# dingodb/dingo-store

Hardware: AMD Instinct MI355X
Metric: QPS @ recall@10, IVF-Flat 10Mx768 nprobe=32 (higher is better)
Workload: dtype f32; 1 GPU; IVF-Flat 10M x 768 fp32 nlist=4096 nprobe=32 batch=1024 k=10; n=10000000, d=768, nlist=4096, nprobe=32, batch=1024, k=10, parallelism=single GPU

## Files before the change

### dingo-store_amd/csrc/dg_abi.cpp

```cpp
#include <cmath>
#include <cstdarg>
#include <cstdio>
#include <cstring>
#include <algorithm>
#include <functional>
#include <atomic>
#include <vector>

#include "dg_internal.h"
#include "dg_sq8_core.h"

static thread_local char g_err[1024] = "";

void dg_set_error(const char* fmt, ...) {
  va_list ap;
  va_start(ap, fmt);
  vsnprintf(g_err, sizeof(g_err), fmt, ap);
  va_end(ap);
}

extern "C" void dg_last_error(char* buf, int64_t len) {
  if (buf && len > 0) {
    strncpy(buf, g_err, len - 1);
    buf[len - 1] = 0;
// ... 20 lines not shown
  }
  g_alloc_gen.fetch_add(1, std::memory_order_relaxed);
  size_t newcap = std::max(bytes, b.cap + b.cap / 2);
  void* np = nullptr;
  if (hipMalloc(&np, newcap) != hipSuccess) {
    dg_set_error("hipMalloc(%zu) failed", newcap);
    return DG_ENOMEM;
  }
  if (keep && b.p && b.bytes) {
    if (hipMemcpyAsync(np, b.p, b.bytes, hipMemcpyDeviceToDevice, s) !=
        hipSuccess) {
      (void)hipFree(np);
      dg_set_error("grow copy failed");
      return DG_EINTERNAL;
    }
  }
  if (b.p) {
    (void)hipStreamSynchronize(s);
    (void)hipFree(b.p);
  }
  b.p = np;
  b.cap = newcap;
  b.bytes = bytes;
  return DG_OK;
}

static bool scan_fused_enabled() {
  const char* e = getenv("DG_SCAN_FUSED");
  return !(e && e[0] == '0' && e[1] == '\0');
}

static bool scan_mfma_enabled() {
  const char* e = getenv("DG_SCAN_MFMA");
  return !(e && e[0] == '0' && e[1] == '\0');
}

static int32_t scan_pair_py() {
  const char* e = getenv("DG_SCAN_PAIR");
  if (e && e[0] && e[1] == '\0') {
    if (e[0] == '0') return 0;
    if (e[0] == '1' || e[0] == '2' || e[0] == '4') return e[0] - '0';
  }
  return dg_index::kScanPairPY;
}

static int32_t scan_f16_py(int32_t mean_probes) {
  const char* e = getenv("DG_SCAN_F16_PY");
  if (e && e[0] && e[1] == '\0' &&
      (e[0] == '1' || e[0] == '2' || e[0] == '4'))
    return e[0] - '0';
  return std::min(4, std::max(1, (mean_probes + 7) / 8));
}

static int64_t range_span_blocks() {
  const char* e = getenv("DG_RANGE_SPAN_BLOCKS");
  const long long v = e ? atoll(e) : 0;
  return v > 0 ? std::min<long long>(v, 1ll << 30) : 1ll << 30;
}

static void dbuf_free(dg_dbuf& b) {
  if (b.p) (void)hipFree(b.p);
  b = {};
}

struct DbufGuard {
  dg_dbuf& b;
// ... 1994 lines not shown
    }
    if (!ix->capturing) (void)hipEventRecord(ix->ev[3], ix->stream);
    if (st == DG_OK) {
      uint64_t* result = slab;
      if (slab_k > k) {
        dgk::fill_base_total(ix->stream, nq, slab_k, bt, bt + nq);
        dgk::select_u64(ix->stream, slab, bt, bt + nq, nq, k, final_tk, k);
        result = final_tk;
      }
      dgk::emit_results(ix->stream, result, (const int64_t*)ix->d_csr_ids.p,
                        dqn, nq, k, emit_metric,
                        metric == DG_METRIC_L2 ? 1 : 0, d_out_dist,
                        d_out_ids);
    }
    if (!ix->capturing) (void)hipEventRecord(ix->ev[4], ix->stream);
    ix->times.last_scan_bytes_alg =
        is_bin ? (int64_t)ix->ntotal * (ix->d_user / 8)
               : (int64_t)ix->ntotal * (d * 4 + 4);
  } else {
    int32_t np = nprobe > 0 ? nprobe : 80;
    np = std::min(np, nlist);
    if ((st = dbuf_reserve(ix->ws_dots, (size_t)nq * nlist * 4, ix->stream,
                           false)) != DG_OK ||
        (st = dbuf_reserve(ix->ws_probes,
                           (size_t)nq * np * 12 + (size_t)nq * k * 8,
                           ix->stream, false)) != DG_OK) {
      return st;
    }
    uint64_t* coarse_tk = (uint64_t*)ix->ws_probes.p;
    int32_t* probes = (int32_t*)(coarse_tk + (size_t)nq * np);
    uint64_t* final_tk = (uint64_t*)(probes + (size_t)nq * np);
    const uint8_t* maskp =
        ix->has_mask ? (const uint8_t*)ix->d_list_mask.p : nullptr;
    if (is_pq && np == nlist) {
      st = sgemm_dots(ix, dq, nq, (const float*)ix->d_centroids.p, nlist, d,
                      (float*)ix->ws_dots.p);
      if (st != DG_OK) {
        return st;
      }
    }
    if (np == nlist) {
      dgk::probes_all(ix->stream, nq, np, maskp, probes);
    } else {
      if (np > 2048) {
        dg_set_error("nprobe %d > 2048 (and < nlist) unsupported", np);
        return DG_ENOT_SUPPORT;
      }
      st = dots(dq, nq, ix->d_centroids.p, nlist, (float*)ix->ws_dots.p);
      if (st != DG_OK) {
        return st;
      }
      const int cmode = is_bin ? 0 : metric == DG_METRIC_L2 ? 1 : 2;
      const int32_t nseg_c = (int32_t)std::min<int64_t>(
          16, std::max<int64_t>(1, nlist / 8192));
      if (nseg_c > 1) {
        dg_dbuf& seg = ix->ws_seg;
        if ((st = dbuf_reserve(seg,
                               (size_t)nq * nseg_c * np * 8 +
                                   (size_t)nq * 2 * 8,
                               ix->stream, false)) != DG_OK)
          return st;
        uint64_t* seg_slab = (uint64_t*)seg.p;
        int64_t* bt_c = (int64_t*)(seg_slab + (size_t)nq * nseg_c * np);
        dgk::select_dense(ix->stream, (const float*)ix->ws_dots.p,
                          (const float*)ix->d_cnorms.p, nq, nlist, nlist,
                          nseg_c, np, cmode, nullptr, 0, seg_slab,
                          (int64_t)nseg_c * np, 0);
        dgk::fill_base_total(ix->stream, nq, (int64_t)nseg_c * np, bt_c,
                             bt_c + nq);
        dgk::select_u64(ix->stream, seg_slab, bt_c, bt_c + nq, nq, np,
                        coarse_tk, np);
      } else {
        dgk::select_dense(ix->stream, (const float*)ix->ws_dots.p,
                          (const float*)ix->d_cnorms.p, nq, nlist, nlist, 1,
                          np, cmode, nullptr, 0, coarse_tk, np, 0);
      }
      dgk::probe_unpack(ix->stream, coarse_tk, nq, np, maskp, probes);
    }
    if (!ix->capturing) (void)hipEventRecord(ix->ev[1], ix->stream);

    size_t inv_bytes = (size_t)nlist * 4 * 3 + ((size_t)nlist + 1) * 12 +
                       (size_t)nq * np * 8 * 2 + ((size_t)nq + 1) * 8 * 2 +
                       (size_t)nq * np * 8 + 64;
    if ((st = dbuf_reserve(ix->ws_inv, inv_bytes, ix->stream, false)) !=
        DG_OK) {
      return st;
    }
    char* wp = (char*)ix->ws_inv.p;
    int32_t* inv_counts = (int32_t*)wp;            wp += (size_t)nlist * 4;
    int32_t* cursors = (int32_t*)wp;               wp += (size_t)nlist * 4;
    wp += (size_t)nlist * 4;
    int64_t* inv_offsets64 = (int64_t*)wp;         wp += ((size_t)nlist + 1) * 8;
    int32_t* inv_offsets32 = (int32_t*)wp;         wp += ((size_t)nlist + 1) * 4;
    int32_t* inv_q = (int32_t*)wp;                 wp += (size_t)nq * np * 4;
    int32_t* inv_rank = (int32_t*)wp;              wp += (size_t)nq * np * 4;
    int64_t* qp_off = (int64_t*)wp;                wp += (size_t)nq * np * 8;
    int64_t* q_total = (int64_t*)wp;               wp += (size_t)nq * 8;
    int64_t* q_cand_base = (int64_t*)wp;

    int64_t* sscr = scan_scratch(ix, &st);
    if (st != DG_OK) {
      return st;
    }
    (void)hipMemsetAsync(inv_counts, 0, (size_t)nlist * 4, ix->stream);
    dgk::hist_probes(ix->stream, probes, nq, np, nlist, inv_counts);
    dgk::excl_scan_i32_to_i64(ix->stream, inv_counts, nlist, inv_offsets64,
                              sscr);
    dgk::init_cursors(ix->stream, inv_offsets64, nlist + 1, inv_offsets32);
    dgk::init_cursors(ix->stream, inv_offsets64, nlist, cursors);
    dgk::scatter_probes(ix->stream, probes, nq, np, nullptr, cursors, inv_q,
                        inv_rank);
    const int32_t chunk_rows = dg_index::kChunkRows;
    const int64_t ub_cand =
        nq * ix->h_len_prefix_desc[std::min<int32_t>(np, nlist)];
    const int64_t partial_per_q =
        (int64_t)np * ix->cpl_max * (chunk_rows / 256) * k;
    const bool fused = !is_pq && !is_bin && !rr &&
                       k <= dg_index::kScanFuseMaxK &&
                       nq * partial_per_q <= ub_cand && scan_fused_enabled();
    ix->last_scan_fused = fused;
    const bool is_f16 = !is_pq && !is_bin && ix->storage == DG_STORAGE_F16;
    ix->last_scan_f16 = is_f16;
    const bool is_sq8 = !is_pq && !is_bin && ix->storage == DG_STORAGE_SQ8;
    ix->last_scan_sq8 = is_sq8;
    if (is_sq8 &&
        (st = dbuf_reserve(ix->ws_sq8q, (size_t)nq * d * 4 + (size_t)nq * 4,
                           ix->stream, false)) != DG_OK)
      return st;
    const bool mfma = fused && (is_f16 || is_sq8 || scan_mfma_enabled());
    ix->last_scan_mfma = mfma;
    const int32_t pair_py =
        mfma && !is_f16 && !is_sq8 && dg_scan_pair_applies((int32_t)d, nq)
            ? scan_pair_py()
            : 0;
    ix->last_scan_pair = pair_py > 0;
    if (pair_py > 0 &&
        (st = dbuf_reserve(ix->ws_qimage,
                           (size_t)dg_scan_qimage_bytes(nq, (int32_t)d),
                           ix->stream, false)) != DG_OK) {
      return st;
    }
    if (fused) {
// ... 130 lines not shown
                          inv_offsets32, inv_q, inv_rank, qp_off, q_cand_base,
                          np, metric, d_bitmap, chunk_rows,
                          (uint64_t*)ix->ws_cand.p, mean_probes);
    }
    if (!ix->capturing) (void)hipEventRecord(ix->ev[3], ix->stream);

    if (rr) {
      if ((st = build_thr(is_bin)) == DG_OK) {
        dgk::count_below(ix->stream, (const uint64_t*)ix->ws_cand.p,
                         q_cand_base, q_total, d_thr, emit_metric, dqn,
                         rr->radius, nq, d_rcounts);
        st = range_finish([&](const int64_t*, int64_t* d_cursors,
                              uint64_t* d_out) -> dg_status {
          dg_dbuf d_off2{};
          dg_status s3 = dbuf_reserve(d_off2, ((size_t)nq + 1) * 8,
                                      ix->stream, false);
          if (s3 != DG_OK) return s3;
          (void)hipMemcpyAsync(d_off2.p, rr->lims, ((size_t)nq + 1) * 8,
                               hipMemcpyHostToDevice, ix->stream);
          dgk::compact_below(ix->stream, (const uint64_t*)ix->ws_cand.p,
                             q_cand_base, q_total, d_thr, emit_metric, dqn,
                             rr->radius, (const int64_t*)d_off2.p, nq,
                             d_cursors, d_out);
          (void)hipStreamSynchronize(ix->stream);
          dbuf_free(d_off2);
          return DG_OK;
        });
      }
      (void)hipEventRecord(ix->ev[4], ix->stream);
      ix->times.last_nq = nq;
      return st;
    }
    if (fused) {
      dgk::fill_base_total(ix->stream, nq, partial_per_q, q_cand_base,
                           q_total);
      dgk::select_u64(ix->stream, (const uint64_t*)ix->ws_partial.p,
                      q_cand_base, q_total, nq, k, final_tk, k);
    } else {
      dgk::select_u64(ix->stream, (const uint64_t*)ix->ws_cand.p, q_cand_base,
                      q_total, nq, k, final_tk, k);
    }
    dgk::emit_results(ix->stream, final_tk, (const int64_t*)ix->d_csr_ids.p,
                      dqn, nq, k, emit_metric, metric == DG_METRIC_L2 ? 1 : 0,
                      d_out_dist, d_out_ids);
    if (!ix->capturing) (void)hipEventRecord(ix->ev[4], ix->stream);
  }
  ix->times.last_nq = nq;
  return st;
}


static dg_status search_device_impl(dg_index* ix, int64_t nq,
                                    const float* d_x, int32_t k,
                                    int32_t nprobe, const dg_filter* filter,
                                    float* d_out_dist, int64_t* d_out_ids,
                                    bool binary_entry, const char* fn,
                                    bool may_capture = true) {
  if (!ix || !d_x || !d_out_dist || !d_out_ids || nq <= 0) {
    dg_set_error("bad search args");
    return DG_EINVAL;
  }
  if (!entry_matches(ix, binary_entry, fn)) return DG_EINVAL;
  if (binary_entry && nq > kMaxScanLen) {
    dg_set_error("nq %lld > %d per call unsupported", (long long)nq,
                 kMaxScanLen);
    return DG_EINVAL;
  }
  if (k <= 0) return DG_OK;
  if (k > 2048) {
    dg_set_error("k > 2048 not supported");
// ... 3 lines not shown
  if (!ix->is_ready() || ix->ntotal == 0 ||
      (ix->desc.kind == DG_INDEX_IVF_PQ && !ix->pq_trained)) {
    std::shared_lock lk(ix->rw);
    (void)hipMemsetAsync(d_out_dist, 0, (size_t)nq * k * 4, ix->stream);
    (void)hipMemsetAsync(d_out_ids, 0xff, (size_t)nq * k * 8, ix->stream);
    return DG_OK;
  }
  {
    std::unique_lock lk(ix->rw, std::defer_lock);
    if (!ix->csr_valid) {
      lk.lock();
      if (!ix->csr_valid) {
        dg_status st = finalize_csr(ix);
        if (st != DG_OK) return st;
      }
    }
  }
  std::shared_lock lk(ix->rw);
  std::lock_guard sg(ix->search_mu);

  const bool graph_ok = nq <= 4 && k <= 128 &&
                        ix->desc.kind == DG_INDEX_IVF_FLAT &&
                        (!filter || filter->kind == DG_FILTER_NONE) &&
                        getenv("DG_NO_GRAPH") == nullptr;
  if (graph_ok) {
    const uint64_t gen =
        ix->index_gen + g_alloc_gen.load(std::memory_order_relaxed);
    const size_t q_bytes = (size_t)nq * ix->d_user * 4;
    const size_t dist_bytes = (size_t)nq * k * 4;
    const size_t ids_bytes = (size_t)nq * k * 8;
    const bool fused_now = scan_fused_enabled();
    const bool mfma_now = scan_mfma_enabled();
    const int32_t pair_now = scan_pair_py();
    if (ix->graph_exec && ix->graph_nq == (int32_t)nq &&
        ix->graph_k == k && ix->graph_np == nprobe &&
        ix->graph_fused == fused_now && ix->graph_mfma == mfma_now &&
        ix->graph_pair == pair_now &&
        ix->graph_gen == gen) {
      DG_HIP_CHECK(hipMemcpyAsync(ix->ws_gq.p, d_x, q_bytes,
                                  hipMemcpyDeviceToDevice, ix->stream));
      DG_HIP_CHECK(hipGraphLaunch(ix->graph_exec, ix->stream));
      DG_HIP_CHECK(hipMemcpyAsync(d_out_dist, ix->ws_gout.p, dist_bytes,
                                  hipMemcpyDeviceToDevice, ix->stream));
      DG_HIP_CHECK(hipMemcpyAsync(
          d_out_ids, (char*)ix->ws_gout.p + dist_bytes, ids_bytes,
          hipMemcpyDeviceToDevice, ix->stream));
      ix->times.last_nq = 0;
      return DG_OK;
    }
    if (!may_capture)
      return search_core(ix, nq, d_x, k, nprobe, filter, d_out_dist,
                         d_out_ids);
    dg_status st = search_core(ix, nq, d_x, k, nprobe, filter, d_out_dist,
                               d_out_ids);
    if (st != DG_OK) return st;
    if (dbuf_reserve(ix->ws_gq, q_bytes, ix->stream, false) != DG_OK ||
        dbuf_reserve(ix->ws_gout, dist_bytes + ids_bytes, ix->stream,
                     false) != DG_OK)
      return DG_OK;
    if (ix->graph_exec) {
      (void)hipGraphExecDestroy(ix->graph_exec);
      ix->graph_exec = nullptr;
    }
    std::unique_lock cl(ix->capture_mu);
    (void)hipStreamSynchronize(ix->stream);
    const uint64_t gen2 =
        ix->index_gen + g_alloc_gen.load(std::memory_order_relaxed);
    ix->capturing = true;
    hipGraph_t graph = nullptr;
    bool captured = false;
    if (hipStreamBeginCapture(ix->stream, hipStreamCaptureModeThreadLocal) ==
        hipSuccess) {
      dg_status cst = search_core(
          ix, nq, (const float*)ix->ws_gq.p, k, nprobe, nullptr,
          (float*)ix->ws_gout.p,
          (int64_t*)((char*)ix->ws_gout.p + dist_bytes));
      if (hipStreamEndCapture(ix->stream, &graph) == hipSuccess &&
          cst == DG_OK && graph) {
        hipGraphExec_t ge = nullptr;
        if (hipGraphInstantiate(&ge, graph, nullptr, nullptr, 0) ==
            hipSuccess) {
          ix->graph_exec = ge;
          ix->graph_nq = (int32_t)nq;
          ix->graph_k = k;
          ix->graph_np = nprobe;
          ix->graph_fused = fused_now;
          ix->graph_mfma = mfma_now;
          ix->graph_pair = pair_now;
          ix->graph_gen = gen2;
          captured = true;
        }
      }
      if (graph) (void)hipGraphDestroy(graph);
    }
    if (!captured) (void)hipGetLastError();
    ix->capturing = false;
    return DG_OK;
  }
  return search_core(ix, nq, d_x, k, nprobe, filter, d_out_dist, d_out_ids);
}

extern "C" dg_status dg_search_device(dg_index* ix, int64_t nq,
                                      const float* d_x, int32_t k,
                                      int32_t nprobe, const dg_filter* filter,
                                      float* d_out_dist, int64_t* d_out_ids) {
  return search_device_impl(ix, nq, d_x, k, nprobe, filter, d_out_dist,
                            d_out_ids, false, "dg_search_device");
}

extern "C" dg_status dg_search_binary_device(dg_index* ix, int64_t nq,
                                             const uint8_t* d_x, int32_t k,
                                             int32_t nprobe,
                                             const dg_filter* filter,
                                             float* d_out_dist,
                                             int64_t* d_out_ids) {
  return search_device_impl(ix, nq, (const float*)d_x, k, nprobe, filter,
                            d_out_dist, d_out_ids, true,
                            "dg_search_binary_device");
}

dg_status dg_search_device_flush(dg_index* ix, int64_t nq, const void* d_x,
// ... 449 lines not shown
        for (size_t i = 0; i < c && st == DG_OK; i++)
          if (ibuf[i] >= 0) ix->id_count.emplace(ibuf[i], 1);
      }
      ix->ntotal = ntotal;
      ix->n_deleted = ndel;
      ix->csr_valid = false;
  ix->index_gen++;
    }
  } while (0);
  fclose(f);
  if (st != DG_OK) {
    dg_index_destroy(ix);
    return st;
  }
  ix->trained = trained != 0;
  *out = ix;
  return DG_OK;
}

extern "C" void dg_lock_write(dg_index* ix) {
  if (ix) ix->rw.lock();
}

extern "C" void dg_unlock_write(dg_index* ix) {
  if (ix) ix->rw.unlock();
}

extern "C" int dg_last_scan_fused(dg_index* ix) {
  if (!ix) return 0;
  std::lock_guard sg(ix->search_mu);
  return ix->last_scan_fused ? 1 : 0;
}

extern "C" int dg_last_scan_pair(dg_index* ix) {
  if (!ix) return 0;
  std::lock_guard sg(ix->search_mu);
  return ix->last_scan_pair ? 1 : 0;
}

extern "C" int dg_last_scan_sq8(dg_index* ix) {
  if (!ix) return 0;
  std::lock_guard sg(ix->search_mu);
  return ix->last_scan_sq8 ? 1 : 0;
}

extern "C" int dg_last_scan_mfma(dg_index* ix) {
  if (!ix) return 0;
  std::lock_guard sg(ix->search_mu);
  return ix->last_scan_mfma ? 1 : 0;
}

extern "C" dg_status dg_stats(dg_index* ix, dg_stats_out* out) {
  if (!ix || !out) return DG_EINVAL;
  std::shared_lock lk(ix->rw);
  DeviceGuard g(ix->device);
  memset(out, 0, sizeof(*out));
  out->ntotal = ix->ntotal - ix->n_deleted;
  out->d = ix->d_user;
  out->metric = ix->desc.metric;
  out->kind = ix->desc.kind;
  out->nlist = ix->desc.nlist;
  out->is_trained = ix->is_ready() ? 1 : 0;
  size_t db = 0;
  for (auto b : {&ix->d_vectors, &ix->d_ids, &ix->d_assign, &ix->d_centroids,
                 &ix->d_cnorms, &ix->d_csr_offsets, &ix->d_csr_vectors,
                 &ix->d_csr_ids, &ix->d_csr_vnorms, &ix->d_csr_t,
// ... 35 lines not shown
```

### dingo-store_amd/csrc/dg_internal.h

```cpp
#pragma once

#include <hip/hip_fp16.h>
#include <hip/hip_runtime.h>
#include <rocblas/rocblas.h>

#include <atomic>
#include <cstdint>
#include <cstdio>
#include <mutex>
#include <shared_mutex>
#include <string>
#include <unordered_map>
#include <vector>

#include "../../include/dingo_gpu.h"
#include "dg_scan_split.h"

#define DG_HIP_CHECK(expr)                                              \
  do {                                                                  \
    hipError_t _e = (expr);                                             \
    if (_e != hipSuccess) {                                             \
      dg_set_error("HIP error %s at %s:%d: %s", hipGetErrorName(_e),    \
                   __FILE__, __LINE__, hipGetErrorString(_e));          \
      return DG_EINTERNAL;                                              \
    }                                                                   \
  } while (0)

#define DG_ROCBLAS_CHECK(expr)                                          \
  do {                                                                  \
    rocblas_status _s = (expr);                                         \
    if (_s != rocblas_status_success) {                                 \
      dg_set_error("rocBLAS error %d at %s:%d", (int)_s, __FILE__,      \
                   __LINE__);                                           \
      return DG_EINTERNAL;                                              \
    }                                                                   \
  } while (0)

void dg_set_error(const char* fmt, ...);

dg_status dg_ingest_rows(dg_index* ix, int64_t n, const int64_t* ids,
                         const float* x, const uint8_t* codes,
                         const int32_t* assign);

dg_status dg_ingest_bits(dg_index* ix, int64_t n, const int64_t* ids,
                         const uint8_t* bits, const int32_t* assign);

dg_status dg_search_device_flush(dg_index* ix, int64_t nq, const void* d_x,
                                 int32_t k, int32_t nprobe,
// ... 84 lines not shown
  dg_dbuf d_csr_t;
  dg_dbuf d_chunk_meta;
  int32_t total_chunks = 0;
  static constexpr int32_t kChunkRows = 1024;
  static constexpr int32_t kScanFuseMaxK = 64;
  static constexpr int32_t kScanPairPY = 2;
  int32_t cpl_max = 0;


  bool pq_trained = false;
  dg_dbuf d_codebooks;
  dg_dbuf d_codes;
  dg_dbuf d_csr_codes;
  dg_dbuf d_S;
  dg_dbuf d_cb_norms;
  dg_dbuf ws_T;
  dg_dbuf ws_Tf32;

  dg_dbuf d_list_mask;
  bool has_mask = false;

  std::unordered_map<int64_t, int32_t> id_count;

  dg_dbuf ws_queries, ws_qnorms, ws_dots, ws_probes, ws_inv, ws_cand,
      ws_units, ws_small, ws_topk;
  dg_dbuf ws_scan;
  dg_dbuf ws_seg;
  dg_dbuf ws_bm;
  dg_dbuf ws_partial;
  bool last_scan_fused = false;
  bool last_scan_mfma = false;
  bool last_scan_pair = false;
  dg_dbuf ws_qimage;

  hipEvent_t ev[12] = {};
  dg_stage_times times;
  bool events_ready = false;

  hipGraphExec_t graph_exec = nullptr;
  int32_t graph_nq = 0, graph_k = 0, graph_np = 0;
  bool graph_fused = false;
  bool graph_mfma = false;
  int32_t graph_pair = 0;
  uint64_t graph_gen = 0;
  uint64_t index_gen = 1;
  dg_dbuf ws_gq, ws_gout;
  bool capturing = false;

  std::atomic<dg_batcher*> batcher{nullptr};

  std::shared_mutex rw;
  std::mutex search_mu;
  std::shared_mutex capture_mu;
};

namespace dgk {
void probe_unpack(hipStream_t s, const uint64_t* topk, int64_t nq,
                  int32_t nprobe, const uint8_t* mask, int32_t* probes);
void probes_all(hipStream_t s, int64_t nq, int32_t nprobe,
                const uint8_t* mask, int32_t* probes);
void init_cursors(hipStream_t s, const int64_t* offsets, int32_t n,
                  int32_t* cursors);
void select_dense(hipStream_t s, const float* scores, const float* cnorms,
                  int64_t rows, int64_t cols, int64_t ld, int32_t nseg,
                  int32_t k, int mode, const uint32_t* bitmap,
                  int64_t col_base, uint64_t* out, int64_t out_stride,
                  int64_t out_offset);
int select_dense_threads(int32_t k);
void select_u64(hipStream_t s, const uint64_t* cand, const int64_t* base,
                const int64_t* total, int64_t nq, int32_t k, uint64_t* out,
                int64_t out_stride);
void gather_rows_by_index(hipStream_t s, const float* src, const int64_t* idx,
                          int64_t n, int32_t d, float* dst);
void fill_base_total(hipStream_t s, int64_t nq, int64_t len, int64_t* base,
                     int64_t* total);
void tombstone(hipStream_t s, const int64_t* pos, int64_t n, int64_t* ids);
void hamming_dists(hipStream_t s, const uint32_t* X, int64_t nq,
                   const uint32_t* Y, int64_t cols, int32_t wp, float* out,
                   int64_t ld);
void hamming_range(hipStream_t s, bool compact, const uint32_t* X, int64_t nq,
                   const uint32_t* Y, int64_t cols, int32_t wp,
                   const uint32_t* bitmap, int32_t radius, int64_t* counts,
                   const int64_t* lims, int64_t* cursors, uint64_t* out,
                   int64_t max_blocks );
void argmin_score(hipStream_t s, const float* scores, int64_t n, int32_t cols,
                  int32_t* out);
void transpose_chunks_u32(hipStream_t s, const uint32_t* units,
                          int32_t n_units, const int64_t* csr_offsets,
                          const int32_t* chunk_off, const int64_t* chunk_base,
                          const uint32_t* rowmajor, int32_t wp,
                          int32_t chunk_rows, uint32_t* twords);
void bivf_scan(hipStream_t s, const uint32_t* units, int32_t n_units,
               const int64_t* csr_offsets, const int32_t* chunk_off,
               const int64_t* chunk_base, const uint32_t* twords,
               const uint32_t* queries, int32_t wp,
               const int32_t* inv_offsets, const int32_t* inv_q,
               const int32_t* inv_rank, const int64_t* qp_off,
               const int64_t* q_cand_base, int32_t nprobe,
               const uint32_t* bitmap, int32_t chunk_rows, uint64_t* cand);
void bits_to_pm1(hipStream_t s, const uint32_t* x, int64_t n, int32_t d,
                 int32_t wp, float* out);
void binarise(hipStream_t s, const float* c, int64_t n, int32_t d, int32_t wp,
              uint32_t* out);
void row_norms(hipStream_t s, const float* x, int64_t n, int32_t d,
               float* out);
void normalize_rows(hipStream_t s, float* x, int64_t n, int32_t d);
void argmin_rows(hipStream_t s, const float* dots, const float* cnorms,
                 int64_t n, int32_t nlist, int metric, int32_t* out);
// ... 168 lines not shown
```

### dingo-store_amd/csrc/kernels.hip.cpp

```cpp
#include <hip/hip_fp16.h>
#include <hip/hip_runtime.h>

#include <cstdint>

#include "dg_internal.h"
#include "dg_shard_core.h"
#include "dg_sq8_core.h"

#define WAVE 64

__device__ __forceinline__ uint32_t enc_f32(float x) {
  uint32_t u = __float_as_uint(x);
  return (int32_t)u < 0 ? ~u : (u | 0x80000000u);
}
__device__ __forceinline__ float dec_f32(uint32_t e) {
  uint32_t u = (e & 0x80000000u) ? (e & 0x7fffffffu) : ~e;
  return __uint_as_float(u);
}
__device__ __forceinline__ uint64_t pack_cand(float key, uint32_t row) {
  return ((uint64_t)enc_f32(key) << 32) | row;
}
static constexpr uint64_t kCandEmpty = ~0ull;

__global__ void k_iota_i32(int32_t* p, int64_t n, int32_t v) {
// ... 115 lines not shown
__device__ void topk_merge_block(uint64_t* lds, int32_t k, int32_t cnt,
                                 uint64_t* out_row ) {
  const int T = blockDim.x;
  const int tid = threadIdx.x;
  uint64_t* a = lds;
  uint64_t* b = lds + (size_t)T * k;
  for (int i = cnt; i < k; i++) a[(size_t)tid * k + i] = kCandEmpty;
  __syncthreads();
  int src_is_a = 1;
  for (int step = 1; step < T; step *= 2) {
    uint64_t* s = src_is_a ? a : b;
    uint64_t* d = src_is_a ? b : a;
    if ((tid & (2 * step - 1)) == 0 && tid + step < T) {
      const uint64_t* x = s + (size_t)tid * k;
      const uint64_t* y = s + (size_t)(tid + step) * k;
      uint64_t* o = d + (size_t)tid * k;
      int xi = 0, yi = 0;
      for (int i = 0; i < k; i++)
        o[i] = (yi >= k || (xi < k && x[xi] <= y[yi])) ? x[xi++] : y[yi++];
    } else if ((tid & (2 * step - 1)) == 0) {
      const uint64_t* x = s + (size_t)tid * k;
      uint64_t* o = d + (size_t)tid * k;
      for (int i = 0; i < k; i++) o[i] = x[i];
    }
    src_is_a ^= 1;
    __syncthreads();
  }
  if (tid == 0) {
    uint64_t* s = (src_is_a ? a : b);
    for (int i = 0; i < k; i++) out_row[i] = s[i];
  }
}

__global__ void k_select_dense(const float* __restrict__ scores,
                               const float* __restrict__ cnorms, int64_t rows,
                               int64_t cols, int64_t ld, int64_t seg_w,
                               int32_t k, int mode,
                               const uint32_t* __restrict__ bitmap,
                               int64_t col_base,
                               uint64_t* __restrict__ out,
                               int64_t out_stride, int64_t out_offset) {
  extern __shared__ uint64_t lds[];
  int64_t row = blockIdx.x;
  if (row >= rows) return;
  const int64_t seg_start = (int64_t)blockIdx.y * seg_w;
  const int64_t cseg = min(seg_w, cols - seg_start);
  const float* sr = scores + row * ld + seg_start;
  const float* cn = cnorms + seg_start;
  uint64_t* mine = lds + (size_t)threadIdx.x * k;
  int32_t cnt = 0;
  for (int64_t c = threadIdx.x; c < cseg; c += blockDim.x) {
    if (bitmap) {
      int64_t g = col_base + seg_start + c;
      if (!((bitmap[g >> 5] >> (g & 31)) & 1)) continue;
    }
    float s = sr[c];
    float key = (mode == 0) ? s : (mode == 1) ? cn[c] - 2.0f * s : -s;
    topk_insert(mine, cnt, k,
                pack_cand(key, (uint32_t)(col_base + seg_start + c)));
  }
  topk_merge_block(lds, k, cnt,
                   out + row * out_stride + out_offset + blockIdx.y * k);
}

__global__ void k_select_u64(const uint64_t* __restrict__ cand,
                             const int64_t* __restrict__ base,
                             const int64_t* __restrict__ total, int64_t nq,
                             int32_t k, uint64_t* __restrict__ out,
                             int64_t out_stride) {
  extern __shared__ uint64_t lds[];
  int64_t q = blockIdx.x;
  if (q >= nq) return;
  const uint64_t* seg = cand + (base ? base[q] : q * total[0]);
  int64_t len = base ? total[q] : total[0];
  uint64_t* mine = lds + (size_t)threadIdx.x * k;
  int32_t cnt = 0;
  for (int64_t i = threadIdx.x; i < len; i += blockDim.x)
    topk_insert(mine, cnt, k, seg[i]);
  topk_merge_block(lds, k, cnt, out + q * out_stride);
}

__global__ void k_emit(const uint64_t* __restrict__ topk,
                       const int64_t* __restrict__ ids_lookup,
                       const float* __restrict__ qnorms, int64_t nq, int32_t k,
                       int metric, int add_qnorm, float* __restrict__ out_dist,
                       int64_t* __restrict__ out_ids) {
  int64_t i = (int64_t)blockIdx.x * blockDim.x + threadIdx.x;
  if (i >= nq * k) return;
  int64_t q = i / k;
  uint64_t c = topk[i];
  if (c == kCandEmpty) {
    out_dist[i] = 0.0f;
    out_ids[i] = -1;
    return;
  }
  float key = dec_f32((uint32_t)(c >> 32));
  uint32_t row = (uint32_t)c;
  float dist;
  if (metric == 0) {
    dist = add_qnorm ? key + qnorms[q] : key;
    if (dist < 0.f) dist = 0.f;
  } else {
    dist = -key;
  }
  out_dist[i] = dist;
  out_ids[i] = ids_lookup ? ids_lookup[row] : (int64_t)row;
}
// ... 34 lines not shown
  if (l >= 0 && mask && !mask[l]) l = -1;
  probes[i] = l;
}

__global__ void k_probes_all(int64_t nq, int32_t nprobe, const uint8_t* mask,
                             int32_t* __restrict__ probes) {
  int64_t i = (int64_t)blockIdx.x * blockDim.x + threadIdx.x;
  if (i >= nq * nprobe) return;
  int32_t l = (int32_t)(i % nprobe);
  if (mask && !mask[l]) l = -1;
  probes[i] = l;
}

__global__ void k_hist_probes(const int32_t* __restrict__ probes, int64_t n,
                              int32_t* __restrict__ counts) {
  int64_t i = (int64_t)blockIdx.x * blockDim.x + threadIdx.x;
  if (i >= n) return;
  int32_t l = probes[i];
  if (l >= 0) atomicAdd(&counts[l], 1);
}

__global__ void k_scatter_probes(const int32_t* __restrict__ probes,
                                 int64_t nq, int32_t nprobe,
                                 int32_t* __restrict__ cursors,
                                 int32_t* __restrict__ inv_q,
                                 int32_t* __restrict__ inv_rank) {
  int64_t i = (int64_t)blockIdx.x * blockDim.x + threadIdx.x;
  if (i >= nq * nprobe) return;
  int32_t l = probes[i];
  if (l < 0) return;
  int32_t pos = atomicAdd(&cursors[l], 1);
  inv_q[pos] = (int32_t)(i / nprobe);
  inv_rank[pos] = (int32_t)(i % nprobe);
}

__global__ void k_cand_offsets(const int32_t* __restrict__ probes, int64_t nq,
                               int32_t nprobe,
                               const int64_t* __restrict__ csr_offsets,
                               int64_t* __restrict__ qp_off,
                               int64_t* __restrict__ q_total) {
  int64_t q = (int64_t)blockIdx.x * blockDim.x + threadIdx.x;
  if (q >= nq) return;
  int64_t run = 0;
  for (int32_t p = 0; p < nprobe; p++) {
    qp_off[q * nprobe + p] = run;
    int32_t l = probes[q * nprobe + p];
    if (l >= 0) run += csr_offsets[l + 1] - csr_offsets[l];
  }
  q_total[q] = run;
}

__global__ void k_alg_bytes(const int32_t* __restrict__ inv_counts,
                            const int64_t* __restrict__ csr_offsets,
                            int32_t nlist, int64_t row_bytes,
                            int64_t* __restrict__ out) {
  __shared__ long long lds[256];
  long long acc = 0;
  for (int32_t l = blockIdx.x * blockDim.x + threadIdx.x; l < nlist;
       l += gridDim.x * blockDim.x)
    if (inv_counts[l] > 0)
      acc += (csr_offsets[l + 1] - csr_offsets[l]) * row_bytes;
  lds[threadIdx.x] = acc;
  __syncthreads();
  for (int s = blockDim.x / 2; s; s >>= 1) {
    if (threadIdx.x < s) lds[threadIdx.x] += lds[threadIdx.x + s];
    __syncthreads();
// ... 3210 lines not shown
                       const dg_dev_filter* f, uint32_t* bitmap) {
  int64_t nwords = ceil_div(n, 32);
  hipLaunchKernelGGL(k_build_pass_bitmap, dim3(ceil_div(nwords, 256)),
                     dim3(256), 0, s, ids, n, *f, bitmap);
}

static inline int select_threads(int32_t k) {
  int T = 256;
  while (T > 2 && 2ull * T * k * 8 > (128u << 10)) T >>= 1;
  return T;
}

int select_dense_threads(int32_t k) { return select_threads(k); }

void select_dense(hipStream_t s, const float* scores, const float* cnorms,
                  int64_t rows, int64_t cols, int64_t ld, int32_t nseg,
                  int32_t k, int mode, const uint32_t* bitmap,
                  int64_t col_base, uint64_t* out, int64_t out_stride,
                  int64_t out_offset) {
  int T = select_threads(k);
  size_t lds = 2ull * T * k * 8;
  int64_t seg_w = (cols + nseg - 1) / nseg;
  hipLaunchKernelGGL(k_select_dense, dim3((uint32_t)rows, (uint32_t)nseg),
                     dim3(T), lds, s, scores, cnorms, rows, cols, ld, seg_w,
                     k, mode, bitmap, col_base, out, out_stride, out_offset);
}

void select_u64(hipStream_t s, const uint64_t* cand, const int64_t* base,
                const int64_t* total, int64_t nq, int32_t k, uint64_t* out,
                int64_t out_stride) {
  int T = select_threads(k);
  size_t lds = 2ull * T * k * 8;
  hipLaunchKernelGGL(k_select_u64, dim3((uint32_t)nq), dim3(T), lds, s, cand,
                     base, total, nq, k, out, out_stride);
}

void emit_results(hipStream_t s, const uint64_t* topk,
                  const int64_t* ids_lookup, const float* qnorms, int64_t nq,
                  int32_t k, int metric, int add_qnorm, float* out_dist,
                  int64_t* out_ids) {
  hipLaunchKernelGGL(k_emit, dim3(ceil_div(nq * k, 256)), dim3(256), 0, s,
                     topk, ids_lookup, qnorms, nq, k, metric, add_qnorm,
                     out_dist, out_ids);
}

void merge_lists(hipStream_t s, const float* dists, const int64_t* ids,
                 int32_t n_lists, int64_t nq, int32_t k_in, int32_t k_out,
                 int metric, float* out_dist, int64_t* out_ids) {
  hipLaunchKernelGGL(k_merge_lists,
                     dim3(ceil_div(nq * n_lists * k_in, 256)), dim3(256), 0,
                     s, dists, ids, n_lists, nq, k_in, k_out, (int32_t)metric,
                     out_dist, out_ids);
}

void probes_all(hipStream_t s, int64_t nq, int32_t nprobe,
                const uint8_t* mask, int32_t* probes) {
  hipLaunchKernelGGL(k_probes_all, dim3(ceil_div(nq * nprobe, 256)),
                     dim3(256), 0, s, nq, nprobe, mask, probes);
}

void probe_unpack(hipStream_t s, const uint64_t* topk, int64_t nq,
                  int32_t nprobe, const uint8_t* mask, int32_t* probes) {
  hipLaunchKernelGGL(k_probe_unpack, dim3(ceil_div(nq * nprobe, 256)),
                     dim3(256), 0, s, topk, nq, nprobe, mask, probes);
}

void hist_probes(hipStream_t s, const int32_t* probes, int64_t nq,
// ... 744 lines not shown
```

### dingo-store_amd/dingostore.py

```python
import ctypes as C
import os

import numpy as np

_DIR = os.path.dirname(os.path.abspath(__file__))
_SO = os.path.join(_DIR, "libdingo_gpu.so")

L2, IP, COSINE = 0, 1, 2
FLAT, IVF_FLAT, IVF_PQ = 0, 1, 2
BINARY_FLAT, BINARY_IVF_FLAT = 3, 4
HAMMING = 3
STORAGE_F32, STORAGE_F16, STORAGE_SQ8 = 0, 1, 2
_STORAGE = {"f32": STORAGE_F32, "f16": STORAGE_F16, "sq8": STORAGE_SQ8}


def _storage_code(storage):
    if storage not in _STORAGE:
        raise DgError(
            f"storage must be 'f32', 'f16' or 'sq8', got {storage!r}")
    return _STORAGE[storage]

_f32p = np.ctypeslib.ndpointer(np.float32, flags="C_CONTIGUOUS")
_u8p = np.ctypeslib.ndpointer(np.uint8, flags="C_CONTIGUOUS")
_i64p = np.ctypeslib.ndpointer(np.int64, flags="C_CONTIGUOUS")
# ... 565 lines not shown
        idx.h = h
        st = idx.stats()
        idx.kind, idx.metric = st["kind"], st["metric"]
        idx.d, idx.nlist = st["d"], st["nlist"]
        idx.m, idx.nbits = 0, 8
        if idx.kind == IVF_PQ:
            m, nbits = C.c_int32(), C.c_int32()
            l = lib()
            l.dg_pq_params.argtypes = [C.c_void_p, C.POINTER(C.c_int32),
                                       C.POINTER(C.c_int32)]
            _check(l.dg_pq_params(h, C.byref(m), C.byref(nbits)),
                   "dg_pq_params")
            idx.m, idx.nbits = m.value, nbits.value
        return idx

    def last_scan_fused(self):
        l = lib()
        l.dg_last_scan_fused.argtypes = [C.c_void_p]
        l.dg_last_scan_fused.restype = C.c_int
        return bool(l.dg_last_scan_fused(self.h))

    def last_scan_mfma(self):
        l = lib()
        l.dg_last_scan_mfma.argtypes = [C.c_void_p]
        l.dg_last_scan_mfma.restype = C.c_int
        return bool(l.dg_last_scan_mfma(self.h))

    def last_scan_pair(self):
        l = lib()
        l.dg_last_scan_pair.argtypes = [C.c_void_p]
        l.dg_last_scan_pair.restype = C.c_int
        return bool(l.dg_last_scan_pair(self.h))

    def stats(self):
        s = _Stats()
        _check(lib().dg_stats(self.h, C.byref(s)), "dg_stats")
        return {f[0]: getattr(s, f[0]) for f in _Stats._fields_
                if not f[0].startswith("_")}


def merge_topk(dists, ids, k, metric=L2):
    dists = np.asarray(dists)
    ids = np.asarray(ids)
    S, nq, kk = dists.shape
    cat_d = dists.transpose(1, 0, 2).reshape(nq, S * kk)
    cat_i = ids.transpose(1, 0, 2).reshape(nq, S * kk)
    key = cat_d if metric == L2 else -cat_d
    key = np.where(cat_i < 0, np.inf, key)
    order = np.lexsort((cat_i, key), axis=1)[:, :k]
    return (np.take_along_axis(cat_d, order, 1),
            np.take_along_axis(cat_i, order, 1))


def merge_topk_device(dists, ids, k, metric=L2, device=-1):
    d = np.ascontiguousarray(dists, np.float32)
    i = np.ascontiguousarray(ids, np.int64)
    if d.ndim != 3 or d.shape != i.shape:
        raise DgError(f"dists / ids must be [n_lists, nq, k_in], got "
                      f"{d.shape} and {i.shape}")
    n_lists, nq, k_in = d.shape
    od = np.empty((nq, k), np.float32)
    oi = np.empty((nq, k), np.int64)
    _check(lib().dg_merge_topk(n_lists, nq, k_in, k, metric, d, i, od, oi,
                               device), "dg_merge_topk")
    return od, oi

# ... 178 lines not shown
```

### include/dingo_gpu.h

```cpp
#ifndef DINGO_GPU_H_
#define DINGO_GPU_H_

#include <stdint.h>

#ifdef __cplusplus
extern "C" {
#endif

typedef enum dg_status {
  DG_OK = 0,
  DG_EINVAL = 1,
  DG_ENOT_TRAINED = 2,
  DG_ENOT_SUPPORT = 3,
  DG_ENOMEM = 4,
  DG_EINTERNAL = 5,
  DG_EIO = 6,
  DG_ENOGPU = 7,
  DG_EID_DUPLICATED = 8,
  DG_ENOT_FOUND = 9
} dg_status;

typedef enum dg_index_kind {
  DG_INDEX_FLAT = 0,
  DG_INDEX_IVF_FLAT = 1,
// ... 196 lines not shown
dg_status dg_sharded_search(dg_sharded* sh, int64_t nq, const float* x,
                            int32_t k, int32_t nprobe,
                            const dg_filter* filter,
                            float* out_dist ,
                            int64_t* out_ids );
dg_status dg_sharded_search_device(dg_sharded* sh, int64_t nq,
                                   const float* d_x, int32_t k,
                                   int32_t nprobe, const dg_filter* filter,
                                   float* d_out_dist, int64_t* d_out_ids);
dg_status dg_sharded_sync(dg_sharded* sh);
dg_status dg_sharded_range_search(dg_sharded* sh, int64_t nq, const float* x,
                                  float radius, const dg_filter* filter,
                                  int64_t* lims ,
                                  int64_t** out_ids, float** out_dists);
dg_status dg_sharded_stats(dg_sharded* sh, dg_stats_out* out);
int32_t dg_sharded_n_shards(dg_sharded* sh);
dg_index* dg_sharded_shard(dg_sharded* sh, int32_t i);
dg_status dg_sharded_set_storage(dg_sharded* sh, int32_t storage);
dg_status dg_sharded_set_sq_ranges(dg_sharded* sh, const float* vmin,
                                   const float* vdiff);
dg_status dg_sharded_get_sq_ranges(dg_sharded* sh, float* vmin, float* vdiff);

void dg_lock_write(dg_index* idx);
void dg_unlock_write(dg_index* idx);

dg_status dg_stats(dg_index* idx, dg_stats_out* out);
void dg_last_error(char* buf, int64_t len);
int dg_last_scan_fused(dg_index* idx);
int dg_last_scan_mfma(dg_index* idx);

int dg_last_scan_pair(dg_index* idx);
int dg_last_scan_f16(dg_index* idx);
int dg_last_scan_sq8(dg_index* idx);
int dg_device_count(void);
const char* dg_build_info(void);

#ifdef __cplusplus
}
#endif
#endif
```

Before: 171,700 queries/s.

## Fuse coarse top-nprobe selection with probe histogram via block radix select

Replaces the coarse-quantizer select_dense plus probe_unpack plus hist_probes sequence with a single per-query radix-select kernel that writes sorted probes and atomically bumps per-list counts. It also replaces the exclusive scan and two init_cursors launches with one single-block kernel that produces all offset arrays and cursors, and it switches the fused final select to a uniform-length variant so fill_base_total is no longer needed. The goal is fewer kernel launches and less pass-over-memory work in the coarse stage. Debug accessors for probes and a coarse-wave flag are added, and the graph cache key now includes the new toggle.

```diff
diff --git a/dingo-store_amd/csrc/dg_abi.cpp b/dingo-store_amd/csrc/dg_abi.cpp
--- a/dingo-store_amd/csrc/dg_abi.cpp
+++ b/dingo-store_amd/csrc/dg_abi.cpp
@@ -76,6 +76,11 @@
 
 static bool scan_mfma_enabled() {
   const char* e = getenv("DG_SCAN_MFMA");
+  return !(e && e[0] == '0' && e[1] == '\0');
+}
+
+static bool coarse_wave_enabled() {
+  const char* e = getenv("DG_COARSE_WAVE");
   return !(e && e[0] == '0' && e[1] == '\0');
 }
 
@@ -2136,53 +2141,6 @@
     uint64_t* final_tk = (uint64_t*)(probes + (size_t)nq * np);
     const uint8_t* maskp =
         ix->has_mask ? (const uint8_t*)ix->d_list_mask.p : nullptr;
-    if (is_pq && np == nlist) {
-      st = sgemm_dots(ix, dq, nq, (const float*)ix->d_centroids.p, nlist, d,
-                      (float*)ix->ws_dots.p);
-      if (st != DG_OK) {
-        return st;
-      }
-    }
-    if (np == nlist) {
-      dgk::probes_all(ix->stream, nq, np, maskp, probes);
-    } else {
-      if (np > 2048) {
-        dg_set_error("nprobe %d > 2048 (and < nlist) unsupported", np);
-        return DG_ENOT_SUPPORT;
-      }
-      st = dots(dq, nq, ix->d_centroids.p, nlist, (float*)ix->ws_dots.p);
-      if (st != DG_OK) {
-        return st;
-      }
-      const int cmode = is_bin ? 0 : metric == DG_METRIC_L2 ? 1 : 2;
-      const int32_t nseg_c = (int32_t)std::min<int64_t>(
-          16, std::max<int64_t>(1, nlist / 8192));
-      if (nseg_c > 1) {
-        dg_dbuf& seg = ix->ws_seg;
-        if ((st = dbuf_reserve(seg,
-                               (size_t)nq * nseg_c * np * 8 +
-                                   (size_t)nq * 2 * 8,
-                               ix->stream, false)) != DG_OK)
-          return st;
-        uint64_t* seg_slab = (uint64_t*)seg.p;
-        int64_t* bt_c = (int64_t*)(seg_slab + (size_t)nq * nseg_c * np);
-        dgk::select_dense(ix->stream, (const float*)ix->ws_dots.p,
-                          (const float*)ix->d_cnorms.p, nq, nlist, nlist,
-                          nseg_c, np, cmode, nullptr, 0, seg_slab,
-                          (int64_t)nseg_c * np, 0);
-        dgk::fill_base_total(ix->stream, nq, (int64_t)nseg_c * np, bt_c,
-                             bt_c + nq);
-        dgk::select_u64(ix->stream, seg_slab, bt_c, bt_c + nq, nq, np,
-                        coarse_tk, np);
-      } else {
-        dgk::select_dense(ix->stream, (const float*)ix->ws_dots.p,
-                          (const float*)ix->d_cnorms.p, nq, nlist, nlist, 1,
-                          np, cmode, nullptr, 0, coarse_tk, np, 0);
-      }
-      dgk::probe_unpack(ix->stream, coarse_tk, nq, np, maskp, probes);
-    }
-    if (!ix->capturing) (void)hipEventRecord(ix->ev[1], ix->stream);
-
     size_t inv_bytes = (size_t)nlist * 4 * 3 + ((size_t)nlist + 1) * 12 +
                        (size_t)nq * np * 8 * 2 + ((size_t)nq + 1) * 8 * 2 +
                        (size_t)nq * np * 8 + 64;
@@ -2201,17 +2159,74 @@
     int64_t* qp_off = (int64_t*)wp;                wp += (size_t)nq * np * 8;
     int64_t* q_total = (int64_t*)wp;               wp += (size_t)nq * 8;
     int64_t* q_cand_base = (int64_t*)wp;
+    (void)hipMemsetAsync(inv_counts, 0, (size_t)nlist * 4, ix->stream);
+    const bool cwave = dg_coarse_wave_applies(np, nlist) &&
+                       coarse_wave_enabled();
+    ix->last_coarse_wave = cwave;
+    ix->last_probes = probes;
+    ix->last_probes_n = nq * (int64_t)np;
+    if (is_pq && np == nlist) {
+      st = sgemm_dots(ix, dq, nq, (const float*)ix->d_centroids.p, nlist, d,
+                      (float*)ix->ws_dots.p);
+      if (st != DG_OK) {
+        return st;
+      }
+    }
+    if (np == nlist) {
+      dgk::probes_all(ix->stream, nq, np, maskp, probes);
+    } else {
+      if (np > 2048) {
+        dg_set_error("nprobe %d > 2048 (and < nlist) unsupported", np);
+        return DG_ENOT_SUPPORT;
+      }
+      st = dots(dq, nq, ix->d_centroids.p, nlist, (float*)ix->ws_dots.p);
+      if (st != DG_OK) {
+        return st;
+      }
+      const int cmode = is_bin ? 0 : metric == DG_METRIC_L2 ? 1 : 2;
+      const int32_t nseg_c = (int32_t)std::min<int64_t>(
+          16, std::max<int64_t>(1, nlist / 8192));
+      if (cwave) {
+        dgk::coarse_select(ix->stream, (const float*)ix->ws_dots.p,
+                           (const float*)ix->d_cnorms.p, nq, nlist, np, cmode,
+                           maskp, probes, inv_counts);
+      } else if (nseg_c > 1) {
+        dg_dbuf& seg = ix->ws_seg;
+        if ((st = dbuf_reserve(seg, (size_t)nq * nseg_c * np * 8, ix->stream,
+                               false)) != DG_OK)
+          return st;
+        uint64_t* seg_slab = (uint64_t*)seg.p;
+        dgk::select_dense(ix->stream, (const float*)ix->ws_dots.p,
+                          (const float*)ix->d_cnorms.p, nq, nlist, nlist,
+                          nseg_c, np, cmode, nullptr, 0, seg_slab,
+                          (int64_t)nseg_c * np, 0);
+        dgk::select_u64_uniform(ix->stream, seg_slab, (int64_t)nseg_c * np,
+                                nq, np, coarse_tk, np);
+        dgk::probe_unpack(ix->stream, coarse_tk, nq, np, maskp, probes);
+      } else {
+        dgk::select_dense(ix->stream, (const float*)ix->ws_dots.p,
+                          (const float*)ix->d_cnorms.p, nq, nlist, nlist, 1,
+                          np, cmode, nullptr, 0, coarse_tk, np, 0);
+        dgk::probe_unpack(ix->stream, coarse_tk, nq, np, maskp, probes);
+      }
+    }
+    if (!ix->capturing) (void)hipEventRecord(ix->ev[1], ix->stream);
 
     int64_t* sscr = scan_scratch(ix, &st);
     if (st != DG_OK) {
       return st;
     }
-    (void)hipMemsetAsync(inv_counts, 0, (size_t)nlist * 4, ix->stream);
-    dgk::hist_probes(ix->stream, probes, nq, np, nlist, inv_counts);
-    dgk::excl_scan_i32_to_i64(ix->stream, inv_counts, nlist, inv_offsets64,
-                              sscr);
-    dgk::init_cursors(ix->stream, inv_offsets64, nlist + 1, inv_offsets32);
-    dgk::init_cursors(ix->stream, inv_offsets64, nlist, cursors);
+    if (!cwave)
+      dgk::hist_probes(ix->stream, probes, nq, np, nlist, inv_counts);
+    if (dg_inv_offsets_applies(nlist)) {
+      dgk::inv_offsets(ix->stream, inv_counts, nlist, inv_offsets64,
+                       inv_offsets32, cursors);
+    } else {
+      dgk::excl_scan_i32_to_i64(ix->stream, inv_counts, nlist, inv_offsets64,
+                                sscr);
+      dgk::init_cursors(ix->stream, inv_offsets64, nlist + 1, inv_offsets32);
+      dgk::init_cursors(ix->stream, inv_offsets64, nlist, cursors);
+    }
     dgk::scatter_probes(ix->stream, probes, nq, np, nullptr, cursors, inv_q,
                         inv_rank);
     const int32_t chunk_rows = dg_index::kChunkRows;
@@ -2408,10 +2423,8 @@
       return st;
     }
     if (fused) {
-      dgk::fill_base_total(ix->stream, nq, partial_per_q, q_cand_base,
-                           q_total);
-      dgk::select_u64(ix->stream, (const uint64_t*)ix->ws_partial.p,
-                      q_cand_base, q_total, nq, k, final_tk, k);
+      dgk::select_u64_uniform(ix->stream, (const uint64_t*)ix->ws_partial.p,
+                              partial_per_q, nq, k, final_tk, k);
     } else {
       dgk::select_u64(ix->stream, (const uint64_t*)ix->ws_cand.p, q_cand_base,
                       q_total, nq, k, final_tk, k);
@@ -2481,10 +2494,11 @@
     const bool fused_now = scan_fused_enabled();
     const bool mfma_now = scan_mfma_enabled();
     const int32_t pair_now = scan_pair_py();
+    const bool cwave_now = coarse_wave_enabled();
     if (ix->graph_exec && ix->graph_nq == (int32_t)nq &&
         ix->graph_k == k && ix->graph_np == nprobe &&
         ix->graph_fused == fused_now && ix->graph_mfma == mfma_now &&
-        ix->graph_pair == pair_now &&
+        ix->graph_pair == pair_now && ix->graph_cwave == cwave_now &&
         ix->graph_gen == gen) {
       DG_HIP_CHECK(hipMemcpyAsync(ix->ws_gq.p, d_x, q_bytes,
                                   hipMemcpyDeviceToDevice, ix->stream));
@@ -2536,6 +2550,7 @@
           ix->graph_fused = fused_now;
           ix->graph_mfma = mfma_now;
           ix->graph_pair = pair_now;
+          ix->graph_cwave = cwave_now;
           ix->graph_gen = gen2;
           captured = true;
         }
@@ -3051,6 +3066,30 @@
   return ix->last_scan_fused ? 1 : 0;
 }
 
+extern "C" int dg_last_coarse_wave(dg_index* ix) {
+  if (!ix) return 0;
+  std::lock_guard sg(ix->search_mu);
+  return ix->last_coarse_wave ? 1 : 0;
+}
+
+extern "C" int64_t dg_last_probes(dg_index* ix, int32_t* out, int64_t n) {
+  if (!ix || n < 0 || (n > 0 && !out)) {
+    dg_set_error("bad dg_last_probes args");
+    return -1;
+  }
+  DeviceGuard g(ix->device);
+  std::lock_guard sg(ix->search_mu);
+  if (!ix->last_probes) return 0;
+  const int64_t m = std::min(n, ix->last_probes_n);
+  if (m > 0 && (hipStreamSynchronize(ix->stream) != hipSuccess ||
+                hipMemcpy(out, ix->last_probes, (size_t)m * 4,
+                          hipMemcpyDeviceToHost) != hipSuccess)) {
+    dg_set_error("dg_last_probes copy failed");
+    return -1;
+  }
+  return ix->last_probes_n;
+}
+
 extern "C" int dg_last_scan_pair(dg_index* ix) {
   if (!ix) return 0;
   std::lock_guard sg(ix->search_mu);
diff --git a/dingo-store_amd/csrc/dg_coarse_wave.h b/dingo-store_amd/csrc/dg_coarse_wave.h
--- /dev/null
+++ b/dingo-store_amd/csrc/dg_coarse_wave.h
@@ -0,0 +1,20 @@
+#pragma once
+#include <cstdint>
+
+constexpr int32_t kCoarseWaveMaxNp = 128;
+constexpr int32_t kCoarseWaveThreads = 256;
+
+constexpr bool dg_coarse_wave_applies(int32_t np, int32_t nlist) {
+  return np >= 1 && np < nlist && np <= kCoarseWaveMaxNp;
+}
+
+constexpr int32_t kInvOffsetsThreads = 1024;
+constexpr int32_t kInvOffsetsMaxNlist = 65536;
+
+constexpr bool dg_inv_offsets_applies(int32_t nlist) {
+  return nlist >= 1 && nlist <= kInvOffsetsMaxNlist;
+}
+
+constexpr int32_t dg_inv_offsets_per_thread(int32_t nlist) {
+  return (nlist + kInvOffsetsThreads - 1) / kInvOffsetsThreads;
+}
diff --git a/dingo-store_amd/csrc/dg_internal.h b/dingo-store_amd/csrc/dg_internal.h
--- a/dingo-store_amd/csrc/dg_internal.h
+++ b/dingo-store_amd/csrc/dg_internal.h
@@ -14,6 +14,7 @@
 #include <vector>
 
 #include "../../include/dingo_gpu.h"
+#include "dg_coarse_wave.h"
 #include "dg_scan_split.h"
 
 #define DG_HIP_CHECK(expr)                                              \
@@ -164,6 +165,9 @@
   bool last_scan_mfma = false;
   bool last_scan_pair = false;
   dg_dbuf ws_qimage;
+  bool last_coarse_wave = false;
+  const int32_t* last_probes = nullptr;
+  int64_t last_probes_n = 0;
 
   hipEvent_t ev[12] = {};
   dg_stage_times times;
@@ -174,6 +178,7 @@
   bool graph_fused = false;
   bool graph_mfma = false;
   int32_t graph_pair = 0;
+  bool graph_cwave = false;
   uint64_t graph_gen = 0;
   uint64_t index_gen = 1;
   dg_dbuf ws_gq, ws_gout;
@@ -206,6 +211,14 @@
                           int64_t n, int32_t d, float* dst);
 void fill_base_total(hipStream_t s, int64_t nq, int64_t len, int64_t* base,
                      int64_t* total);
+void select_u64_uniform(hipStream_t s, const uint64_t* cand, int64_t len,
+                        int64_t nq, int32_t k, uint64_t* out,
+                        int64_t out_stride);
+void coarse_select(hipStream_t s, const float* dots, const float* cnorms,
+                   int64_t nq, int32_t nlist, int32_t np, int mode,
+                   const uint8_t* mask, int32_t* probes, int32_t* counts);
+void inv_offsets(hipStream_t s, const int32_t* counts, int32_t nlist,
+                 int64_t* off64, int32_t* off32, int32_t* cursors);
 void tombstone(hipStream_t s, const int64_t* pos, int64_t n, int64_t* ids);
 void hamming_dists(hipStream_t s, const uint32_t* X, int64_t nq,
                    const uint32_t* Y, int64_t cols, int32_t wp, float* out,
diff --git a/dingo-store_amd/csrc/kernels.hip.cpp b/dingo-store_amd/csrc/kernels.hip.cpp
--- a/dingo-store_amd/csrc/kernels.hip.cpp
+++ b/dingo-store_amd/csrc/kernels.hip.cpp
@@ -171,6 +171,15 @@
   }
 }
 
+__device__ __forceinline__ float select_key_v(int mode, float cn, float s) {
+  return (mode == 0) ? s : (mode == 1) ? cn - 2.0f * s : -s;
+}
+__device__ __forceinline__ float select_key(int mode,
+                                            const float* __restrict__ cn,
+                                            int64_t c, float s) {
+  return select_key_v(mode, mode == 1 ? cn[c] : 0.0f, s);
+}
+
 __global__ void k_select_dense(const float* __restrict__ scores,
                                const float* __restrict__ cnorms, int64_t rows,
                                int64_t cols, int64_t ld, int64_t seg_w,
@@ -193,8 +202,7 @@
       int64_t g = col_base + seg_start + c;
       if (!((bitmap[g >> 5] >> (g & 31)) & 1)) continue;
     }
-    float s = sr[c];
-    float key = (mode == 0) ? s : (mode == 1) ? cn[c] - 2.0f * s : -s;
+    float key = select_key(mode, cn, c, sr[c]);
     topk_insert(mine, cnt, k,
                 pack_cand(key, (uint32_t)(col_base + seg_start + c)));
   }
@@ -204,14 +212,16 @@
 
 __global__ void k_select_u64(const uint64_t* __restrict__ cand,
                              const int64_t* __restrict__ base,
-                             const int64_t* __restrict__ total, int64_t nq,
-                             int32_t k, uint64_t* __restrict__ out,
+                             const int64_t* __restrict__ total, int64_t ulen,
+                             int64_t nq, int32_t k,
+                             uint64_t* __restrict__ out,
                              int64_t out_stride) {
   extern __shared__ uint64_t lds[];
   int64_t q = blockIdx.x;
   if (q >= nq) return;
-  const uint64_t* seg = cand + (base ? base[q] : q * total[0]);
-  int64_t len = base ? total[q] : total[0];
+  const uint64_t* seg =
+      cand + (ulen >= 0 ? q * ulen : base ? base[q] : q * total[0]);
+  int64_t len = ulen >= 0 ? ulen : base ? total[q] : total[0];
   uint64_t* mine = lds + (size_t)threadIdx.x * k;
   int32_t cnt = 0;
   for (int64_t i = threadIdx.x; i < len; i += blockDim.x)
@@ -312,6 +322,133 @@
   int32_t pos = atomicAdd(&cursors[l], 1);
   inv_q[pos] = (int32_t)(i / nprobe);
   inv_rank[pos] = (int32_t)(i % nprobe);
+}
+
+__global__ void __launch_bounds__(kCoarseWaveThreads)
+k_coarse_select(const float* __restrict__ dots,
+                const float* __restrict__ cnorms, int32_t nlist, int32_t np,
+                int mode, const uint8_t* __restrict__ mask,
+                int32_t* __restrict__ probes, int32_t* __restrict__ counts) {
+  __shared__ uint32_t hist[256];
+  __shared__ uint64_t surv[kCoarseWaveMaxNp];
+  __shared__ uint32_t s_bin, s_need, s_done, s_cnt;
+  const int tid = threadIdx.x, lane = tid & (WAVE - 1);
+  const int64_t q = blockIdx.x;
+  const float* row = dots + q * nlist;
+  const int32_t n4 = (nlist & 3) == 0 ? nlist >> 2 : 0;
+
+  auto for_each_key = [&](auto&& f) {
+    for (int32_t g = tid; g < n4; g += kCoarseWaveThreads) {
+      const float4 s = ((const float4*)row)[g];
+      float4 c = {0.f, 0.f, 0.f, 0.f};
+      if (mode == 1) c = ((const float4*)cnorms)[g];
+      const uint32_t col = 4u * (uint32_t)g;
+      f(pack_cand(select_key_v(mode, c.x, s.x), col));
+      f(pack_cand(select_key_v(mode, c.y, s.y), col + 1));
+      f(pack_cand(select_key_v(mode, c.z, s.z), col + 2));
+      f(pack_cand(select_key_v(mode, c.w, s.w), col + 3));
+    }
+    for (int32_t c = 4 * n4 + tid; c < nlist; c += kCoarseWaveThreads)
+      f(pack_cand(select_key(mode, cnorms, c, row[c]), (uint32_t)c));
+  };
+
+  uint64_t prefix = 0;
+  uint32_t need = (uint32_t)np;
+  int shift = 56;
+  for (int b = 7; b >= 0; b--) {
+    if (b > 0 && b < 4 && ((uint32_t)(nlist - 1) >> (8 * b)) == 0) continue;
+    shift = 8 * b;
+    hist[tid] = 0;
+    if (tid == 0) s_cnt = 0;
+    __syncthreads();
+    for_each_key([&](uint64_t key) {
+      if (b == 7 || (key >> (shift + 8)) == (prefix >> (shift + 8))) {
+        const uint32_t bin = (uint32_t)(key >> shift) & 255u;
+        const uint32_t first = __builtin_amdgcn_readfirstlane(bin);
+        const uint64_t act = __ballot(1);
+        if (__ballot(bin == first) == act) {
+          if (lane == __ffsll((long long)act) - 1)
+            atomicAdd(&hist[first], (uint32_t)__popcll(act));
+        } else {
+          atomicAdd(&hist[bin], 1u);
+        }
+      }
+    });
+    __syncthreads();
+    if (tid < WAVE) {
+      const uint32_t h0 = hist[4 * lane], h1 = hist[4 * lane + 1],
+                     h2 = hist[4 * lane + 2], h3 = hist[4 * lane + 3];
+      const uint32_t sum = h0 + h1 + h2 + h3;
+      uint32_t incl = sum;
+      for (int off = 1; off < WAVE; off <<= 1) {
+        const uint32_t t = __shfl_up(incl, off, WAVE);
+        if (lane >= off) incl += t;
+      }
+      const uint32_t excl = incl - sum;
+      if (excl < need && need <= incl) {
+        uint32_t r = need - excl, j = 0, hj = h0;
+        if (r > hj) { r -= hj; j = 1; hj = h1; }
+        if (r > hj) { r -= hj; j = 2; hj = h2; }
+        if (r > hj) { r -= hj; j = 3; hj = h3; }
+        s_bin = 4 * lane + j;
+        s_need = r;
+        s_done = (hj == r) ? 1u : 0u;
+      }
+    }
+    __syncthreads();
+    prefix |= (uint64_t)s_bin << shift;
+    need = s_need;
+    if (s_done) break;
+  }
+
+  const uint64_t limit = prefix >> shift;
+  for_each_key([&](uint64_t key) {
+    if ((key >> shift) <= limit) {
+      const uint32_t slot = atomicAdd(&s_cnt, 1u);
+      if (slot < (uint32_t)np) surv[slot] = key;
+    }
+  });
+  __syncthreads();
+  if (tid < np) {
+    const uint64_t key = surv[tid];
+    int32_t rank = 0;
+    for (int32_t j = 0; j < np; j++) rank += surv[j] < key ? 1 : 0;
+    int32_t l = (int32_t)(key & 0xffffffffu);
+    if (mask && !mask[l]) l = -1;
+    probes[q * np + rank] = l;
+    if (l >= 0) atomicAdd(&counts[l], 1);
+  }
+}
+
+__global__ void __launch_bounds__(kInvOffsetsThreads)
+k_inv_offsets(const int32_t* __restrict__ counts, int32_t nlist,
+              int64_t* __restrict__ off64, int32_t* __restrict__ off32,
+              int32_t* __restrict__ cursors) {
+  __shared__ int64_t wsum[kInvOffsetsThreads / WAVE];
+  const int tid = threadIdx.x, lane = tid & (WAVE - 1), w = tid / WAVE;
+  const int32_t per = dg_inv_offsets_per_thread(nlist);
+  const int32_t lo = min(tid * per, nlist), hi = min(lo + per, nlist);
+  int64_t sum = 0;
+  for (int32_t i = lo; i < hi; i++) sum += counts[i];
+  int64_t incl = sum;
+  for (int off = 1; off < WAVE; off <<= 1) {
+    const int64_t t = __shfl_up(incl, off, WAVE);
+    if (lane >= off) incl += t;
+  }
+  if (lane == WAVE - 1) wsum[w] = incl;
+  __syncthreads();
+  int64_t run = incl - sum;
+  for (int i = 0; i < w; i++) run += wsum[i];
+  for (int32_t i = lo; i < hi; i++) {
+    off64[i] = run;
+    off32[i] = (int32_t)run;
+    cursors[i] = (int32_t)run;
+    run += counts[i];
+  }
+  if (tid == kInvOffsetsThreads - 1) {
+    off64[nlist] = run;
+    off32[nlist] = (int32_t)run;
+  }
 }
 
 __global__ void k_cand_offsets(const int32_t* __restrict__ probes, int64_t nq,
@@ -3588,7 +3725,31 @@
   int T = select_threads(k);
   size_t lds = 2ull * T * k * 8;
   hipLaunchKernelGGL(k_select_u64, dim3((uint32_t)nq), dim3(T), lds, s, cand,
-                     base, total, nq, k, out, out_stride);
+                     base, total, (int64_t)-1, nq, k, out, out_stride);
+}
+
+void select_u64_uniform(hipStream_t s, const uint64_t* cand, int64_t len,
+                        int64_t nq, int32_t k, uint64_t* out,
+                        int64_t out_stride) {
+  int T = select_threads(k);
+  size_t lds = 2ull * T * k * 8;
+  hipLaunchKernelGGL(k_select_u64, dim3((uint32_t)nq), dim3(T), lds, s, cand,
+                     (const int64_t*)nullptr, (const int64_t*)nullptr, len,
+                     nq, k, out, out_stride);
+}
+
+void coarse_select(hipStream_t s, const float* dots, const float* cnorms,
+                   int64_t nq, int32_t nlist, int32_t np, int mode,
+                   const uint8_t* mask, int32_t* probes, int32_t* counts) {
+  hipLaunchKernelGGL(k_coarse_select, dim3((uint32_t)nq),
+                     dim3(kCoarseWaveThreads), 0, s, dots, cnorms, nlist, np,
+                     mode, mask, probes, counts);
+}
+
+void inv_offsets(hipStream_t s, const int32_t* counts, int32_t nlist,
+                 int64_t* off64, int32_t* off32, int32_t* cursors) {
+  hipLaunchKernelGGL(k_inv_offsets, dim3(1), dim3(kInvOffsetsThreads), 0, s,
+                     counts, nlist, off64, off32, cursors);
 }
 
 void emit_results(hipStream_t s, const uint64_t* topk,
diff --git a/dingo-store_amd/dingostore.py b/dingo-store_amd/dingostore.py
--- a/dingo-store_amd/dingostore.py
+++ b/dingo-store_amd/dingostore.py
@@ -621,6 +621,21 @@
         l.dg_last_scan_pair.restype = C.c_int
         return bool(l.dg_last_scan_pair(self.h))
 
+    def last_coarse_wave(self):
+        l = lib()
+        l.dg_last_coarse_wave.argtypes = [C.c_void_p]
+        l.dg_last_coarse_wave.restype = C.c_int
+        return bool(l.dg_last_coarse_wave(self.h))
+
+    def last_probes(self):
+        l = lib()
+        l.dg_last_probes.argtypes = [C.c_void_p, C.c_void_p, C.c_int64]
+        l.dg_last_probes.restype = C.c_int64
+        out = np.empty(max(l.dg_last_probes(self.h, None, 0), 0), np.int32)
+        if l.dg_last_probes(self.h, out.ctypes.data, out.size) != out.size:
+            raise DgError("dg_last_probes: " + last_error())
+        return out
+
     def stats(self):
         s = _Stats()
         _check(lib().dg_stats(self.h, C.byref(s)), "dg_stats")
diff --git a/include/dingo_gpu.h b/include/dingo_gpu.h
--- a/include/dingo_gpu.h
+++ b/include/dingo_gpu.h
@@ -252,6 +252,8 @@
 int dg_last_scan_pair(dg_index* idx);
 int dg_last_scan_f16(dg_index* idx);
 int dg_last_scan_sq8(dg_index* idx);
+int dg_last_coarse_wave(dg_index* idx);
+int64_t dg_last_probes(dg_index* idx, int32_t* out, int64_t n);
 int dg_device_count(void);
 const char* dg_build_info(void);
 
```

New measurement: 180,900 queries/s (median of 6 runs). +5.4%, better.
